# qwerty35/swarm_simulator

Hardware: AMD Instinct MI355X
Metric: agent-trajectories/sec (RBP plan: SFC+RSFC+QP) (higher is better)
Workload: dtype f64

## Files before the change

__graft_entry__.py:

```python
import os
import subprocess
import sys

ROOT = os.path.dirname(os.path.abspath(__file__))
if ROOT not in sys.path:
    sys.path.insert(0, ROOT)


def build() -> None:
    env = dict(os.environ)
    env.setdefault("PYTORCH_ROCM_ARCH", "gfx950")
    subprocess.check_call(["make", "-C", os.path.join(ROOT, "swarm_simulator_amd", "csrc"), "all", "prof", "dev", "chain"], env=env)
    subprocess.check_call(["make", "-C", os.path.join(ROOT, "oracle"), "all"], env=env)
    rocm = os.environ.get("ROCM_PATH", "/opt/rocm")
    if os.path.exists(os.path.join(rocm, "include", "rccl", "rccl.h")):
        try:
            subprocess.check_call(["make", "-C", os.path.join(ROOT, "swarm_simulator_amd", "csrc", "rccl"), "all", f"ROCM={rocm}"], env=env)
        except subprocess.CalledProcessError as e:
            print("build: WARNING: lib/librbp_rccl.so (the optional RCCL exchange hook) did not build:", e)
    else:
        print("build: no RCCL headers under", rocm, "-- lib/librbp_rccl.so (the optional RCCL exchange hook) is not built")
    import swarm_simulator_amd
    from swarm_simulator_amd import host, planner
    host.lib()
    L = planner.lib()
    for name in planner.EXPORTED_SYMBOLS:
        getattr(L, name)
    print("build ok:", L.rbp_version().decode())


def smoke() -> None:
    import numpy as np
    from swarm_simulator_amd import host, planner
    from swarm_simulator_amd.types import Param
    from tests import oracle_lib as O

    if planner.lib().rbp_device_count() < 1:
        raise RuntimeError("smoke(): no HIP device visible; the RBP path has no CPU fallback")
    p = Param.test_sweep()
    m = host.load_mission("mission_64agents_15.json").subset([0, 16, 32, 48, 8, 24, 40, 56])
    w = host.load_world("map1.bt", p)
    init = host.ecbs_plan(w, m, p)
    ref, gpu = init.clone_inputs(), init.clone_inputs()
    rc, _ = O.corridor_update(w, m, p, ref)
    assert rc == 0
    cor = planner.Corridor(w, m, p)
    assert cor.update(False, gpu), cor.last_error
    assert np.array_equal(ref.sfc_box, gpu.sfc_box) and np.array_equal(ref.sfc_count, gpu.sfc_count)
    assert np.array_equal(ref.rsfc_normal.view(np.uint32), gpu.rsfc_normal.view(np.uint32))
    rc, rep = O.planner_update(m, p, ref)
    assert rc == 0
    pl = planner.RBPPlanner(m, p)
    assert pl.update(False, gpu), pl.last_error
    err = float(np.abs(ref.ctrl - gpu.ctrl).max())
    rel = abs(ref.total_cost - gpu.total_cost) / max(1.0, abs(ref.total_cost))
    print(f"smoke: N={m.qn} M={gpu.M} cost gpu={gpu.total_cost:.9f} oracle={ref.total_cost:.9f} "
          f"ctrl sup-err={err:.2e} rel cost err={rel:.2e}")
    assert err < 1e-5 and rel < 1e-7, (err, rel)
    print("smoke ok")


if __name__ == "__main__":
    build()
    if len(sys.argv) > 1 and sys.argv[1] == "smoke":
        smoke()
```

swarm_simulator_amd/csrc/kernels/knot_lds.inc:

```
#pragma once
#include "knot_panel_layout.h"

#define KL_LD 38
#define KL_LDU 50
#define KL_I 40
#ifndef KL_XCH
#define KL_XCH 6
#endif
typedef __attribute__((address_space(3))) double kl_lds;
typedef __attribute__((address_space(3))) int kl_ldsi;
typedef double kl_d2 __attribute__((ext_vector_type(2)));
typedef __attribute__((address_space(3))) kl_d2 kl_lds2;
typedef double kl_d4 __attribute__((ext_vector_type(4)));

__host__ __device__ constexpr int kl_area_doubles(int nk) {
    return ((nk + 1) * KL_LDU + (nk + 1) * KL_LD + KL_I + 1) & ~1;
}

template <int NK>
struct KlArea {
    static constexpr int NT = (NK + 15) / 16;
    static constexpr int C = 0, CSZ = (NK + 1) * KL_LDU;
    static constexpr int MX = CSZ, MXSZ = (NK + 1) * KL_LD;
    static constexpr int I = MX + MXSZ;
// ... 459 lines not shown

template <int NK, bool WAIT>
__device__ __forceinline__ void kl_inverse_panels(kl_d4 (&n)[KlPanels<NK>::TILES], const kl_lds* C, int lane, kl_ldsi* P, int pbase) {
    constexpr int NT = KlPanels<NK>::NT, NP = KlPanels<NK>::NP;
    const int li = lane & 15, lk = lane >> 4;
#pragma unroll
    for (int ti = 0; ti < NT; ++ti)
#pragma unroll
        for (int tj = 0; tj <= ti; ++tj)
#pragma unroll
            for (int g = 0; g < 4; ++g) n[kp_lower(ti, tj)][g] = (ti == tj && lk + 4 * g == li) ? 1.0 : 0.0;
#pragma unroll
    for (int p = 0; p < NP; ++p) {
        const int tc = kp_panel_tile(p), q = kp_panel_reg(p);
        if (WAIT) kl_await_opaque(P, pbase + p + 1);
        const kl_lds* img = C + kp_img_off(NK, p);
        const kl_lds* bl = img + kp_img_entry(KP_W * p, 0);
        const double l10 = bl[4], l32 = bl[14];
        const kl_d2 r2 = *(const kl_lds2*)(bl + 8), r3 = *(const kl_lds2*)(bl + 12);
        kl_d2 raw[NT][2];
        kl_rows_load<NK>(raw, img, tc, li);
        const double l20 = r2[0], l21 = r2[1], l30 = r3[0], l31 = r3[1];
        const double k10 = -l10, k21 = -l21, k32 = -l32;
        const double k20 = __builtin_fma(-l21, k10, -l20), k31 = __builtin_fma(-l32, k21, -l31);
        const double k30 = __builtin_fma(-l32, k20, __builtin_fma(-l31, k10, -l30));
        double a[NT], b[NT];
#pragma unroll
        for (int t = 0; t < NT; ++t)
            if (t >= tc) {
                const double L[4] = {raw[t][0][0], raw[t][0][1], raw[t][1][0], raw[t][1][1]};
                double G[4];
                G[3] = -L[3];
                G[2] = -__builtin_fma(L[3], k32, L[2]);
                G[1] = -__builtin_fma(L[3], k31, __builtin_fma(L[2], k21, L[1]));
                G[0] = -__builtin_fma(L[3], k30, __builtin_fma(L[2], k20, __builtin_fma(L[1], k10, L[0])));
                if (t == tc) {
                    const int ar = KP_T * t + li - KP_W * p;
                    G[0] = kl_pick(ar >= 4, G[0], kl_pick(ar == 1, k10, kl_pick(ar == 2, k20, kl_pick(ar == 3, k30, 0.0))));
                    G[1] = kl_pick(ar >= 4, G[1], kl_pick(ar == 2, k21, kl_pick(ar == 3, k31, 0.0)));
                    G[2] = kl_pick(ar >= 4, G[2], kl_pick(ar == 3, k32, 0.0));
                    G[3] = kl_pick(ar >= 4, G[3], 0.0);
                }
                a[t] = kl_sel4(G, lk);
            }
#pragma unroll
        for (int tj = 0; tj < NT; ++tj)
            if (tj <= tc) b[tj] = n[kp_lower(tc, tj)][q];
#pragma unroll
        for (int ti = 0; ti < NT; ++ti)
#pragma unroll
            for (int tj = 0; tj <= ti; ++tj)
                if (ti >= tc && tj <= tc) n[kp_lower(ti, tj)] = __builtin_amdgcn_mfma_f64_16x16x4f64(a[ti], b[tj], n[kp_lower(ti, tj)], 0, 0, 0);
    }
}

template <int NK>
__device__ __forceinline__ void kl_tiles_scatter(const kl_d4 (&n)[KlPanels<NK>::TILES], kl_lds* MX, int lane) {
    constexpr int NT = KlPanels<NK>::NT;
    const int li = lane & 15, lk = lane >> 4;
#pragma unroll
    for (int ti = 0; ti < NT; ++ti)
#pragma unroll
        for (int tj = 0; tj < NT; ++tj)
#pragma unroll
            for (int g = 0; g < 4; ++g) {
                if (KP_T * ti + 4 * g >= NK) continue;
                const int col = KP_T * ti + lk + 4 * g, row = KP_T * tj + li;
                const bool in = (KP_T * tj + KP_T <= NK || row < NK) && (KP_T * ti + 4 * g + 4 <= NK || col < NK);
                MX[in ? row * KL_LD + col : NK * KL_LD + li] = tj <= ti ? n[kp_lower(ti, tj)][g] : 0.0;
            }
    kl_sync();
}
template <int NK>
__device__ __forceinline__ void kl_row_load(double (&m)[NK], const kl_lds* MX, int r, bool act) {
    const kl_lds* row = MX + (act ? r : NK) * KL_LD;
#pragma unroll
    for (int k = 0; k + 1 < NK; k += 2) {
        const kl_d2 t = *(const kl_lds2*)(row + k);
        m[k] = t[0], m[k + 1] = t[1];
    }
    if (NK & 1) m[NK - 1] = row[NK - 1];
}

template <int NK, bool FOLLOW>
__device__ __forceinline__ double kl_inverse_rows(double (&m)[NK], const kl_lds* C, const kl_lds* I, kl_lds* MX, int r, bool act, kl_ldsi* P, int pbase,
                                                  kl_ldsi* Mdone = nullptr, int done_value = 0) {
    if constexpr (kl_panel_path(NK)) {
        kl_d4 n[KlPanels<NK>::TILES];
        kl_inverse_panels<NK, FOLLOW>(n, C, r, P, pbase);
        kl_tiles_scatter<NK>(n, MX, r);
        if (kl_fused_path(NK)) {
            if (FOLLOW) kl_await_opaque(P, pbase + NK + 1);
            const double dinv = I[act ? r : 0];
            __builtin_amdgcn_fence(__ATOMIC_RELEASE, "wavefront");
            if (FOLLOW) kl_publish(Mdone, done_value);
            kl_row_load<NK>(m, MX, r, act);
            return dinv;
        }
        kl_row_load<NK>(m, MX, r, act);
        kl_sync();
        if (FOLLOW) kl_await_opaque(P, pbase + NK + 1);
        const double dinv = I[act ? r : 0];
        if (FOLLOW) kl_publish(Mdone, done_value);
        return dinv;
    } else {
#pragma unroll
        for (int k = 0; k < NK; ++k) m[k] = (k == r) ? 1.0 : 0.0;
        if (FOLLOW)
            kl_follow_LinvT<NK>(m, C, I, P, pbase);
        else
            kl_row_times_LinvT<NK>(m, C, I);
        if (FOLLOW) kl_await_opaque(P, pbase + NK + 1);
        const double dinv = I[act ? r : 0];
        kl_store_rows<NK>(m, MX, r, act);
        if (FOLLOW) kl_publish(Mdone, done_value);
        return dinv;
    }
}

#include "knot_subst.h"
template <int NK>
__device__ __forceinline__ void kl_forward_step(kl_lds* base, __attribute__((address_space(1))) double* z_out, double rhs_r, double e0, double e1, double e2, int r) {
    using A = KlArea<NK>;
    using F = KfSlots<NK>;
    static_assert(F::CSZ == A::CSZ, "knot_subst.h out of step with KlArea");
    kl_lds *C = base + A::C, *MX = base + A::MX, *I = base + A::I;
    const int rr = r < NK ? r : 0, g3 = 3 * (rr / 3);
    ks_step_forward<NK, true>((const kl_lds*)MX, I[rr], rhs_r, true, e0, e1, e2, C + F::A, C + F::Z, C + F::V, C + F::PS, r, g3, rr, [] { kl_sync(); },
                              [&](double z) { *z_out = z; });
}
template <int NK>
__device__ __forceinline__ double kl_middle_step(kl_lds* base, double v, int r) {
    using A = KlArea<NK>;
    using F = KfSlots<NK>;
    kl_lds* C = base + A::C;
    const int rr = r < NK ? r : 0;
    return ks_step_middle<NK, true>((const kl_lds*)(base + A::MX), (const kl_lds*)(base + A::I + rr), v, C + F::A, C + F::Z, C + F::PS, r, rr, [] { kl_sync(); });
}
```

swarm_simulator_amd/csrc/kernels/qp.hip:

```cpp
#include <algorithm>
#include <type_traits>
#include <vector>

#include "rbp_dev.h"

#pragma clang fp contract(fast)

#include "knot_lds.inc"
#include "common/ipm_rows.h"
#include "common/reduce_order.h"

#ifndef QP_THREADS
#define QP_THREADS 512
#endif
#define QP_MAX_ITERS 80
#ifndef QP_WARM_TAU
#define QP_WARM_TAU 1e-3
#endif
#ifndef QP_MU0
#define QP_MU0 3e-1
#endif
#ifndef QP_ROW_UNROLL
#define QP_ROW_UNROLL 2
#endif
#ifndef QP_ROW_PF
#define QP_ROW_PF 0
#endif
#ifndef QP_ROW_BLK
#define QP_ROW_BLK (QP_THREADS >= 512 ? 0 : 4)
#endif
#define QG(p) ((__attribute__((address_space(1))) double*)(p))
#define QGC(p) ((__attribute__((address_space(1))) const double*)(p))
#define QGF(p) ((__attribute__((address_space(1))) const float*)(p))
#ifndef QP_FAR_SLACK
#define QP_FAR_SLACK 0.7
#endif
#ifndef QP_SIGMA_POW
#define QP_SIGMA_POW 3
#endif
#ifndef QP_NBHD_GAMMA
#define QP_NBHD_GAMMA 1e-3
#endif
#ifndef QP_NBHD_BACKOFF
#define QP_NBHD_BACKOFF 0.8
#endif
#ifndef QP_STEP_FRAC
#define QP_STEP_FRAC 0.997
#endif
#ifndef QP_SFLOOR
#define QP_SFLOOR 1e-1
#endif
#ifndef QP_WAVES_PER_EU
#define QP_WAVES_PER_EU 2
#endif
#ifndef QP_CHAIN_PRIO
#define QP_CHAIN_PRIO 3
#endif
#ifndef QP_STAGE_BUFS
#define QP_STAGE_BUFS (QP_THREADS >= 512 ? 3 : 2)
#endif
#ifndef QP_STAGE_REGS
#define QP_STAGE_REGS (QP_THREADS >= 512 ? 0 : 2)
#endif
#ifndef QP_MID_FOLLOW
#define QP_MID_FOLLOW (QP_THREADS >= 512)
#endif
#ifndef QP_LF_PACKED
#define QP_LF_PACKED (QP_THREADS >= 512 ? 0 : 1)
#endif
#ifndef QP_FWD_IN_FACTOR
#ifdef QP_TRACE
#define QP_FWD_IN_FACTOR 0
#else
#define QP_FWD_IN_FACTOR 1
#endif
#endif
#if QP_FWD_IN_FACTOR && KL_FUSED_UPDATE && KL_PANEL && KL_PANEL_MIN_NK <= 36
#define QP_FWD36 1
#else
#define QP_FWD36 0
#endif
#ifndef QP_EARLY_TRIES
#define QP_EARLY_TRIES 2
#endif
#ifndef QP_EARLY_TOL
#define QP_EARLY_TOL 1e-6
#endif
#include "lh_layout.h"
#include "knot_factor_layout.h"
#define PL_NC 256
#define PL_PMAX 160
#define PL_PBIG 192
__host__ __device__ inline int polish_pmax(int nk) { return nk <= 36 ? 112 : PL_PMAX; }
__host__ __device__ inline size_t polish_s_doubles(int nj) { return std::max((size_t)PL_NC * PL_NC, ipm::k0g_doubles(nj)); }
__host__ __device__ inline size_t polish_ws_doubles(int nj, int nk) {
    return 18 * (size_t)nj + 2 + ipm::k0g_doubles(nj) + PL_NC * 14 + polish_s_doubles(nj) + 8 + lhp_size(PL_PBIG) + 4 * 6 * PL_PBIG + 3 * (size_t)nj * nk;
}
__host__ __device__ inline int polish_lds_doubles(int nk) {
    const int pm = polish_pmax(nk);
    return lhp_size(pm) + 3 * PL_NC + 3 * pm + (pm + 2 * PL_NC + 8) / 2 + 8;
}

namespace {
using namespace ipm;

#include "qp_base.inc"
#include "qp_polish_types.inc"
#include "qp_rows.inc"
#include "qp_newton.inc"
#include "qp_wave_factor.inc"
#include "qp_wave_solve.inc"
#include "qp_tiled.inc"
#include "qp_entries.inc"
#include "qp_polish.inc"
#include "qp_batch.inc"

__global__ __launch_bounds__(QP_THREADS, QP_WAVES_PER_EU) void qp_batch_kernel(DevSession S, double* ws_base, size_t ws_stride, int passes,
                                                               int biter, int nbmax, int lds_doubles) {
    const int mission = S.qp_order ? __builtin_amdgcn_readfirstlane(S.qp_order[blockIdx.x]) : (int)blockIdx.x;
    const long long t_start = wall_clock64();
    __shared__ DevSession S_lds;
    if (threadIdx.x == 0) S_lds = S;
    __syncthreads();
    mission_tables(&S_lds, ws_base, ws_stride, mission, nbmax);
    int stop_it = -1, stop_l = 0;
    for (int it = 0; it < passes && stop_it < 0; ++it)
        for (int l = 0; l < biter; ++l) {
            const double far_R = (it == 0 && S.p.polish && S.p.far_slack > 0.0) ? S.p.far_slack : 1e300;
            const int again = qp_batch_body(S, ws_base, ws_stride, mission, l, nbmax, (int)(l == 0), lds_doubles, it, far_R);
            __threadfence_block();
            __syncthreads();
            if (again) {
                stop_it = it, stop_l = l;
                break;
            }
        }
    if (stop_it >= 0) qp_finish_schedule(&S_lds, ws_base, ws_stride, mission, passes, biter, nbmax, lds_doubles, stop_it, stop_l);
    if (S.qp_cost && threadIdx.x == 0) S.qp_cost[mission] = (unsigned long long)(wall_clock64() - t_start) + 1;
}

__global__ __launch_bounds__(256) void qp_order_kernel(DevSession S) {
    const int k = blockIdx.x * blockDim.x + threadIdx.x;
    if (k >= S.K) return;
    const unsigned long long c = S.qp_cost[k];
    int rank = 0;
    bool valid = c != 0;
    for (int o = 0; o < S.K; ++o) {
        const unsigned long long co = S.qp_cost[o];
        valid = valid && co != 0;
        rank += (co > c || (co == c && o < k)) ? 1 : 0;
    }
    if (valid)
        S.qp_order[rank] = k;
    else
        S.qp_order[k] = k;
}

}

#ifndef QP_SUFFIX
#define QP_SUFFIX _w2
#endif
#define QP_CAT2(a, b) a##b
#define QP_CAT(a, b) QP_CAT2(a, b)
size_t QP_CAT(planner_workspace_bytes, QP_SUFFIX)(int N, int M, int batch_size_eff) {
    return (ws_doubles(N, M, batch_size_eff) * sizeof(double) + 255) & ~size_t(255);
}

static size_t qp_lds_bytes(int bs, int M) {
    const int nk = 9 * bs;
    const int nkw = std::min(nk, 36);
    size_t lds = sizeof(double) * (2 * (size_t)((nk + 15) & ~15) + QP_THREADS + 32) + 16;
// ... 34 lines not shown
```

swarm_simulator_amd/csrc/kernels/qp_newton.inc:

```

__device__ void apply_FT(const QpDims& d, const QpWs& w, const double* cvec, double* out, double scale) {
    const int oq = d.oq, nu = 3 * d.nb;
    for (int it = threadIdx.x; it < d.nj * nu; it += QP_THREADS) {
        const int j = it / nu + 1, u = it % nu;
        const double* xr = cvec + (size_t)u * oq + 6 * j;
        const double* xl = cvec + (size_t)u * oq + 6 * (j - 1) + 3;
        const double* L = w.Lk + 9 * j;
#pragma unroll
        for (int e = 0; e < 3; ++e)
            out[(size_t)(j - 1) * d.nk + u * 3 + e] = scale * (xr[e] + L[0 + e] * xl[0] + L[3 + e] * xl[1] + L[6 + e] * xl[2]);
    }
}
__device__ void apply_F(const QpDims& d, const QpWs& w, const double* du, double* dx) {
    const int oq = d.oq, nu = 3 * d.nb;
    for (int it = threadIdx.x; it < d.nj * nu; it += QP_THREADS) {
        const int j = it / nu + 1, u = it % nu;
        const double* uu = du + (size_t)(j - 1) * d.nk + u * 3;
        const double* L = w.Lk + 9 * j;
        const double u0 = uu[0], u1 = uu[1], u2 = uu[2];
        double* o = dx + (size_t)u * oq + 6 * (j - 1) + 3;
        o[0] = L[0] * u0 + L[1] * u1 + L[2] * u2;
        o[1] = L[3] * u0 + L[4] * u1 + L[5] * u2;
        o[2] = L[6] * u0 + L[7] * u1 + L[8] * u2;
        o[3] = u0, o[4] = u1, o[5] = u2;
// ... 62 lines not shown
    }
}
__device__ void rhs_from_acc(const RowCtx& c, bool corrector, double sigma_mu) {
    const QpDims& d = c.d;
    const QpWs& w = c.w;
    const int oq = d.oq, nu = 3 * d.nb;
    for (int it = threadIdx.x; it < d.nj * nu; it += QP_THREADS) {
        const int j = it / nu + 1, u = it % nu, a = u / 3, k = u % 3;
        double g[6];
#pragma unroll
        for (int q = 0; q < 6; ++q) {
            const int j6 = 6 * (j - 1) + 3 + q;
            const double* ac = w.cpacc + (size_t)a * oq + j6;
            const size_t ncp = (size_t)d.nb * oq;
            const double gv = corrector ? ac[k * ncp] - sigma_mu * ac[(3 + k) * ncp] : ac[(6 + k) * ncp];
            g[q] = gv;
        }
        const double* L = w.Lk + 9 * j;
        const size_t o0 = (size_t)(j - 1) * d.nk + u * 3;
#pragma unroll
        for (int e = 0; e < 3; ++e) w.rhs[o0 + e] = w.rbase[o0 + e] + g[3 + e] + L[0 + e] * g[0] + L[3 + e] * g[1] + L[6 + e] * g[2];
    }
}

__device__ inline double sym3s(const double* S, size_t stride, int k, int l) {
    const int a = k < l ? k : l, b = k < l ? l : k;
    return S[(size_t)(a == 0 ? b : (a == 1 ? 2 + b : 5)) * stride];
}
__device__ inline double sym3(const double* S, int k, int l) {
    const int a = k < l ? k : l, b = k < l ? l : k;
    return S[a == 0 ? b : (a == 1 ? 2 + b : 5)];
}

struct AsmArgs {
    const double *cpacc, *pwgt, *Lk, *Dk;
    const float* normals;
    double* Td;
    int N, M, nb, first, oq, ldb;
};
__device__ __forceinline__ AsmArgs uni(const AsmArgs& A) {
    return AsmArgs{uni(A.cpacc), uni(A.pwgt), uni(A.Lk), uni(A.Dk), uni(A.normals), uni(A.Td), uni(A.N), uni(A.M), uni(A.nb), uni(A.first), uni(A.oq), uni(A.ldb)};
}

__device__ __forceinline__ void assemble_load(const AsmArgs& A, const double* Ssum, int j, int a, int b, int k, int l, double (&Sv)[6]) {
    const int nb = A.nb, oq = A.oq;
#pragma unroll
    for (int p = 0; p < 6; ++p) {
        const int j6 = 6 * (j - 1) + 3 + p;
        double sv;
        if (a == b) {
            sv = Ssum ? sym3(Ssum + ((size_t)a * oq + j6) * 6, k, l) : sym3s(A.cpacc + (size_t)a * oq + j6, (size_t)nb * oq, k, l);
        } else {
            const int lo = a < b ? a : b, hi = a < b ? b : a, seg = j6 / 6;
            const float* nv = A.normals + (pair_index(A.N, A.first + lo, A.first + hi) * A.M + seg) * 3;
            sv = -A.pwgt[(size_t)(lo * nb - lo * (lo + 1) / 2 + (hi - lo - 1)) * oq + j6] * (double)nv[k] * (double)nv[l];
        }
        Sv[p] = sv;
    }
}
__device__ __forceinline__ void assemble_store(const AsmArgs& A, int j, int a, int b, int k, int l, const double (&Sv)[6], bool lower_only) {
    const int lb = A.ldb;
    const double* L = A.Lk + 9 * j;
    double* out = A.Td + (size_t)(j - 1) * lb * lb + (size_t)(a * 9 + k * 3) * lb + b * 9 + l * 3;
#pragma unroll
    for (int e = 0; e < 3; ++e)
#pragma unroll
        for (int f = 0; f < 3; ++f) {
            double acc = Sv[0] * L[e] * L[f] + Sv[1] * L[3 + e] * L[3 + f] + Sv[2] * L[6 + e] * L[6 + f];
            if (e == f) acc += Sv[3 + e];
            if (a == b && k == l) acc += A.Dk[9 * j + 3 * e + f];
            if (!(lower_only && a == b && k == l && e > f)) out[(size_t)e * lb + f] = acc;
        }
}
__device__ __forceinline__ void assemble_item(const AsmArgs& A, const double* Ssum, int j, int r, bool lower_only = false) {
    const int nb = A.nb;
    const int a = r / (nb * 9), b = (r / 9) % nb, k = (r / 3) % 3, l = r % 3;
    if (lower_only && (a > b || (a == b && k > l))) return;
    double Sv[6];
    assemble_load(A, Ssum, j, a, b, k, l, Sv);
    assemble_store(A, j, a, b, k, l, Sv, lower_only);
}

#define ASML_DOUBLES(nk, nb) ((nk) * KL_LD + (nb) * 36 + 3 * (nb) * ((nb) - 1) + 3 * (nb) * ((nb) - 1) + 8)
template <bool TO_GLOBAL, class NextFn, class DoneFn>
__device__ __forceinline__ void assemble_knots_lds(const AsmArgs& A, double* scratch, NextFn next, DoneFn done) {
    const int nb = A.nb, oq = A.oq, nk = 9 * nb, npb = nb * (nb - 1) / 2, n3 = 3 * nb, per = n3 * (n3 + 1) / 2;
    const int lane = threadIdx.x & 63;
    const size_t ncp = (size_t)nb * oq;
    kl_lds* Timg = (kl_lds*)scratch;
    kl_lds* Sin = Timg + nk * KL_LD;
    kl_lds* Pw = Sin + nb * 36;
    kl_lds* Nr = Pw + 6 * npb;
    int tA[2], tB[2], ntile = 0;
#pragma unroll
    for (int u = 0; u < 2; ++u) {
        const int t = lane + 64 * u, tc = t < per ? t : 0;
        int ai = (int)(((2 * n3 + 1) - sqrtf((float)((2 * n3 + 1) * (2 * n3 + 1) - 8 * tc))) * 0.5f);
        if (ai * n3 - ai * (ai - 1) / 2 > tc) ai--;
        if ((ai + 1) * n3 - (ai + 1) * ai / 2 <= tc) ai++;
        tA[u] = ai, tB[u] = ai + tc - (ai * n3 - ai * (ai - 1) / 2);
        if (t < per) ntile = u + 1;
    }
    const int row0 = (2 * lane) / nk, col0 = (2 * lane) % nk, drow = 128 / nk, dcol = 128 % nk;
    size_t nr_off = 0;
    if (lane < 6 * npb) {
        const int pw = lane / 6, sg = (lane / 3) % 2, c3 = lane % 3;
        int lo = 0, rest = pw;
        while (rest >= nb - 1 - lo) rest -= nb - 1 - lo, lo++;
        const int hi = lo + 1 + rest;
        nr_off = (pair_index(A.N, A.first + lo, A.first + hi) * A.M + sg) * 3 + c3;
    }
    for (int j = next(); j >= 0; j = next()) {
        const int jn = j + 1, j60 = 6 * j + 3;
        for (int idx = lane; idx < nb * 36; idx += 64) {
            const int a = idx / 36, e = (idx / 6) % 6, pp = idx % 6;
            Sin[idx] = A.cpacc[(size_t)e * ncp + (size_t)a * oq + j60 + pp];
        }
        for (int idx = lane; idx < 6 * npb; idx += 64) Pw[idx] = A.pwgt[(size_t)(idx / 6) * oq + j60 + idx % 6];
        if (lane < 6 * npb) Nr[lane] = (double)A.normals[nr_off + (size_t)j * 3];
        double L[9], Dk[9];
#pragma unroll
        for (int e = 0; e < 9; ++e) L[e] = A.Lk[9 * jn + e], Dk[e] = A.Dk[9 * jn + e];
        kl_sync();
#pragma unroll
        for (int u = 0; u < 2; ++u) {
            if (u < ntile) {
                const int Ai = tA[u], Bi = tB[u], a = Ai / 3, k = Ai % 3, b = Bi / 3, l = Bi % 3;
                double Sv[6];
                if (a == b) {
                    const int kk = k < l ? k : l, ll = k < l ? l : k, sym = kk == 0 ? ll : (kk == 1 ? 2 + ll : 5);
#pragma unroll
                    for (int pp = 0; pp < 6; ++pp) Sv[pp] = Sin[(a * 6 + sym) * 6 + pp];
                } else {
                    const int pw = a * nb - a * (a + 1) / 2 + (b - a - 1);
#pragma unroll
                    for (int pp = 0; pp < 6; ++pp) Sv[pp] = -Pw[pw * 6 + pp] * Nr[(pw * 2 + (pp >= 3)) * 3 + k] * Nr[(pw * 2 + (pp >= 3)) * 3 + l];
                }
#pragma unroll
                for (int e = 0; e < 3; ++e)
#pragma unroll
                    for (int f = 0; f < 3; ++f) {
                        double acc = Sv[0] * L[e] * L[f] + Sv[1] * L[3 + e] * L[3 + f] + Sv[2] * L[6 + e] * L[6 + f];
                        if (e == f) acc += Sv[3 + e];
                        if (Ai == Bi) acc += Dk[3 * e + f];
                        Timg[(3 * Ai + e) * KL_LD + 3 * Bi + f] = acc;
                        Timg[(3 * Bi + f) * KL_LD + 3 * Ai + e] = acc;
                    }
            }
        }
        kl_sync();
        if (TO_GLOBAL) {
            double* Tg = A.Td + (size_t)j * nk * nk;
            if ((nk & 1) == 0) {
                int r = row0, k2 = col0;
                for (int idx = lane; idx < nk * nk / 2; idx += 64) {
                    if (k2 + 1 >= r) *(kl_d2*)(Tg + 2 * idx) = *(const kl_lds2*)(Timg + r * KL_LD + k2);
                    r += drow, k2 += dcol;
                    if (k2 >= nk) k2 -= nk, r++;
                }
            } else {
                for (int idx = lane; idx < nk * nk; idx += 64) Tg[idx] = Timg[(idx / nk) * KL_LD + idx % nk];
            }
        }
        done(j);
        kl_sync();
    }
}
__device__ __noinline__ void fasm_fetch(AsmArgs Av, double* scratch_v, int jv) {
    typedef __attribute__((address_space(1))) const void gvoid;
    typedef __attribute__((address_space(3))) void lvoid;
    typedef __attribute__((address_space(3))) char lchar;
    const AsmArgs A = uni(Av);
    double* scratch = uni(scratch_v);
    const int j = __builtin_amdgcn_readfirstlane(jv);
    const int nb = A.nb, oq = A.oq, nk = 9 * nb, npb = nb * (nb - 1) / 2, lane = threadIdx.x & 63, j60 = 6 * j + 3;
    const size_t ncp = (size_t)nb * oq;
    lchar* Sin = (lchar*)((kl_lds*)scratch + nk * KL_LD);
    lchar* Pw = Sin + (size_t)nb * 36 * 8;
    lchar* Nr = Pw + (size_t)6 * npb * 8;
    asm volatile("s_waitcnt lgkmcnt(0)" ::: "memory");
    for (int c = 0; c * 64 < nb * 72; ++c) {
        const int dw = c * 64 + lane, idx = dw >> 1, a = idx / 36, e = (idx / 6) % 6, pp = idx % 6;
        if (dw < nb * 72)
            __builtin_amdgcn_global_load_lds((gvoid*)((const unsigned*)(A.cpacc + (size_t)e * ncp + (size_t)a * oq + j60 + pp) + (dw & 1)), (lvoid*)(Sin + c * 256), 4, 0, 0);
    }
    for (int c = 0; c * 64 < npb * 12; ++c) {
        const int dw = c * 64 + lane, idx = dw >> 1;
        if (dw < npb * 12)
            __builtin_amdgcn_global_load_lds((gvoid*)((const unsigned*)(A.pwgt + (size_t)(idx / 6) * oq + j60 + idx % 6) + (dw & 1)), (lvoid*)(Pw + c * 256), 4, 0, 0);
    }
    if (lane < 6 * npb) {
        const int pw = lane / 6, sg = (lane / 3) % 2, c3 = lane % 3;
        int lo = 0, rest = pw;
        while (rest >= nb - 1 - lo) rest -= nb - 1 - lo, lo++;
        const int hi = lo + 1 + rest;
        const size_t off = (pair_index(A.N, A.first + lo, A.first + hi) * A.M + sg + j) * 3 + c3;
        __builtin_amdgcn_global_load_lds((gvoid*)(A.normals + off), (lvoid*)Nr, 4, 0, 0);
    }
}
__device__ __noinline__ void fasm_tiles(AsmArgs Av, double* scratch_v, int jv) {
    const AsmArgs A = uni(Av);
    double* scratch = uni(scratch_v);
    const int j = __builtin_amdgcn_readfirstlane(jv);
    const int nb = A.nb, nk = 9 * nb, npb = nb * (nb - 1) / 2, n3 = 3 * nb, per = n3 * (n3 + 1) / 2, lane = threadIdx.x & 63, jn = j + 1;
    kl_lds* Timg = (kl_lds*)scratch;
    const kl_lds* Sin = Timg + nk * KL_LD;
    const kl_lds* Pw = Sin + nb * 36;
    const __attribute__((address_space(3))) float* Nr = (const __attribute__((address_space(3))) float*)(Pw + 6 * npb);
    double L[9], Dk[9];
#pragma unroll
    for (int e = 0; e < 9; ++e) L[e] = A.Lk[9 * jn + e], Dk[e] = A.Dk[9 * jn + e];
    asm volatile("s_waitcnt vmcnt(0)" ::: "memory");
    kl_sync();
    for (int u = 0; u * 64 < per; ++u) {
        const int t = lane + 64 * u;
        if (t < per) {
            int Ai = (int)(((2 * n3 + 1) - sqrtf((float)((2 * n3 + 1) * (2 * n3 + 1) - 8 * t))) * 0.5f);
            if (Ai * n3 - Ai * (Ai - 1) / 2 > t) Ai--;
            if ((Ai + 1) * n3 - (Ai + 1) * Ai / 2 <= t) Ai++;
            const int Bi = Ai + t - (Ai * n3 - Ai * (Ai - 1) / 2);
            const int a = Ai / 3, k = Ai % 3, b = Bi / 3, l = Bi % 3;
            double Sv[6];
            if (a == b) {
                const int kk = k < l ? k : l, ll = k < l ? l : k, sym = kk == 0 ? ll : (kk == 1 ? 2 + ll : 5);
#pragma unroll
                for (int pp = 0; pp < 6; ++pp) Sv[pp] = Sin[(a * 6 + sym) * 6 + pp];
            } else {
                const int pw = a * nb - a * (a + 1) / 2 + (b - a - 1);
#pragma unroll
                for (int pp = 0; pp < 6; ++pp)
                    Sv[pp] = -Pw[pw * 6 + pp] * (double)Nr[(pw * 2 + (pp >= 3)) * 3 + k] * (double)Nr[(pw * 2 + (pp >= 3)) * 3 + l];
            }
#pragma unroll
            for (int e = 0; e < 3; ++e)
#pragma unroll
                for (int f = 0; f < 3; ++f) {
                    double acc = Sv[0] * L[e] * L[f] + Sv[1] * L[3 + e] * L[3 + f] + Sv[2] * L[6 + e] * L[6 + f];
                    if (e == f) acc += Sv[3 + e];
                    if (Ai == Bi) acc += Dk[3 * e + f];
                    Timg[(3 * Ai + e) * KL_LD + 3 * Bi + f] = acc;
                    Timg[(3 * Bi + f) * KL_LD + 3 * Ai + e] = acc;
                }
        }
    }
    kl_sync();
}
__device__ void assemble_blocks_lds(const AsmArgs& A, int nj, double* lds) {
    const int wave = threadIdx.x >> 6, NW = QP_THREADS / 64;
    int j = wave - NW;
    assemble_knots_lds<true>(A, lds + (size_t)wave * ASML_DOUBLES(9 * A.nb, A.nb), [&] { j += NW; return j < nj ? j : -1; }, [](int) {});
}

__device__ inline AsmArgs asm_args(const RowCtx& c) {
    return AsmArgs{c.w.cpacc, c.w.pwgt, c.w.Lk, c.w.Dk, c.normals, c.w.Td, c.d.N, c.d.M, c.d.nb, c.d.first, c.d.oq, c.d.ldb};
}

__device__ void assemble_blocks(const RowCtx& c, double* lds) {
    const QpDims& d = c.d;
    const QpWs& w = c.w;
    const int nk = d.nk, oq = d.oq, nb = d.nb, lb = d.ldb;
    const AsmArgs A = asm_args(c);
    const bool in_lds = nb * oq * 6 <= c.lds_avail;
    if (in_lds) {
        for (int it = threadIdx.x; it < nb * oq * 6; it += QP_THREADS) lds[it] = w.cpacc[(size_t)(it % 6) * (nb * oq) + it / 6];
        __syncthreads();
    }
    const int per_knot = nb * nb * 9;
    for (int it = threadIdx.x; it < d.nj * per_knot; it += QP_THREADS) assemble_item(A, in_lds ? lds : nullptr, it / per_knot + 1, it % per_knot);
    if (d.nj > 1 && nk > 36 && 3 * lb * (lb + 2) > c.lds_avail) {
        const size_t noff = (size_t)(d.nj - 1) * lb * lb;
        for (size_t it = threadIdx.x; it < noff; it += QP_THREADS) {
            const int j = (int)(it / ((size_t)lb * lb)) + 1;
            const int rr = (int)(it % ((size_t)lb * lb)) / lb, cc = (int)(it % ((size_t)lb * lb)) % lb;
            double v = 0;
            if (rr / 3 == cc / 3 && rr < nk && cc < nk) v = w.Ek[9 * j + 3 * (cc % 3) + (rr % 3)];
            w.To[it] = v;
        }
    }
}
```

swarm_simulator_amd/csrc/kernels/qp_wave_factor.inc:

```

__device__ __forceinline__ int twist_mid(int nj) { return nj / 2; }

#define ASM_WAVE0 4
#define ASM_HELPERS (QP_THREADS / 64 > ASM_WAVE0 ? QP_THREADS / 64 - ASM_WAVE0 : 0)
#ifndef QP_FOLLOW_ASM
#define QP_FOLLOW_ASM (ASM_HELPERS == 0)
#endif
#define ASMF_READY(cnt, h) ((kl_ldsi*)((cnt) + 76 + (h)))
__device__ __forceinline__ void wait_blocks(int* cnt, int i) {
    while (__hip_atomic_load(cnt + i, __ATOMIC_RELAXED, __HIP_MEMORY_SCOPE_WORKGROUP) < ASM_HELPERS) __builtin_amdgcn_s_sleep(2);
    __builtin_amdgcn_fence(__ATOMIC_ACQUIRE, "workgroup");
}

typedef double d4 __attribute__((ext_vector_type(4)));

template <int NK>
__device__ __forceinline__ bool chol_rows(double (&a)[NK], double& dinv) {
    bool ok = true;
    const int r = threadIdx.x & 63;
    dinv = 1.0;
#pragma unroll
    for (int c = 0; c < NK; ++c) {
        const double dcc = rl(a[c], c);
        if (!(dcc > 0)) ok = false;
        const double inv = fast_rsqrt(dcc);
        dinv = (r == c) ? inv : dinv;
        a[c] *= inv;
#pragma unroll
        for (int k = c + 1; k < NK; ++k) a[k] -= a[c] * rl(a[c], k);
    }
    return ok;
}

#if QP_LF_PACKED
#define KF_SLOT(NK) kf_stride(NK)
#define KF_ELEM(NK, r, k) kf_elem(NK, r, k)
#define KF_DINV(NK) kf_dinv(NK)
#else
static_assert(KL_I == 40, "kf_sq_stride (knot_factor_layout.h) restates KL_I");
#define KF_SLOT(NK) kf_sq_stride(NK)
#define KF_ELEM(NK, r, k) kf_sq_elem(NK, r, k)
#define KF_DINV(NK) kf_sq_dinv(NK)
#endif
static_assert(KF_SLOT(9) + 15 <= 2 * 81 && KF_SLOT(18) + 15 <= 2 * 324 && KF_SLOT(27) + 15 <= 2 * 729 && KF_SLOT(36) + 15 <= 2 * 1296,
              "a knot's slot and the doubles in front of the first one fit the region carve() gives QpWs::Lf");

__device__ __forceinline__ void coupling_coef(const QpWs& w, int j, int dir, int rr, double& e0, double& e1, double& e2) {
    const __attribute__((address_space(1))) double* E = QGC(w.Ek) + 9 * (dir > 0 ? j + 1 : j);
    e0 = dir > 0 ? E[rr % 3] : E[3 * (rr % 3)], e1 = dir > 0 ? E[3 + rr % 3] : E[3 * (rr % 3) + 1],
    e2 = dir > 0 ? E[6 + rr % 3] : E[3 * (rr % 3) + 2];
}

template <int NK>
__device__ __forceinline__ bool knot_ldl(const QpWs& w, int j, bool minus_u, kl_lds* base, int r, bool act, int rr, kl_ldsi* P, int pbase,
                                         const kl_lds* Timg = nullptr, kl_ldsi* consumed = nullptr, int consumed_value = 0) {
    using A = KlArea<NK>;
    kl_lds *C = base + A::C, *I = base + A::I, *U = base + A::C;
    if constexpr (kl_panel_path(NK)) {
        if (Timg)
            return kl_knot_panels<NK, true>([&](int mx, int mn) { return (double)Timg[mn * KL_LD + mx]; },
                                      [&] {
                                          kl_sync();
                                          if (consumed) kl_publish(consumed, consumed_value);
                                      },
                                      minus_u, C, I, r, P, pbase);
        const double* Tg = w.Td + (size_t)j * NK * NK;
        return kl_knot_panels<NK, false>([&](int mx, int mn) { return Tg[mn * NK + mx]; }, [] {}, minus_u, C, I, r, P, pbase);
    }
    double a[NK];
    if (Timg) {
#pragma unroll
        for (int k = 0; k < NK; ++k) a[k] = Timg[k * KL_LD + rr];
        kl_sync();
        if (consumed) kl_publish(consumed, consumed_value);
    } else {
        const double* Tg = w.Td + (size_t)j * NK * NK;
#pragma unroll
        for (int k = 0; k < NK; ++k) a[k] = Tg[k * NK + rr];
    }
    if (minus_u) {
#pragma unroll
        for (int k = 0; k < NK; ++k) a[k] -= U[rr * KL_LDU + k];
        kl_sync();
    }
    return kl_ldl<NK>(a, C, I, r, act, P, pbase);
}

template <int NK>
__device__ __forceinline__ bool knot_ldl_add(const QpWs& w, int j, kl_d4 (&s)[KlPanels<NK>::TILES], kl_lds* base, int r, kl_ldsi* P, int pbase,
                                             const kl_lds* Timg = nullptr, kl_ldsi* consumed = nullptr, int consumed_value = 0) {
    using A = KlArea<NK>;
    kl_lds *C = base + A::C, *I = base + A::I;
    if (Timg)
        return kl_knot_panels_add<NK, true>(s, [&](int mx, int mn) { return (double)Timg[mn * KL_LD + mx]; },
                                            [&] {
                                                kl_sync();
                                                if (consumed) kl_publish(consumed, consumed_value);
                                            },
                                            C, I, r, P, pbase);
    const double* Tg = w.Td + (size_t)j * NK * NK;
    return kl_knot_panels_add<NK, false>(s, [&](int mx, int mn) { return Tg[mn * NK + mx]; }, [] {}, C, I, r, P, pbase);
}
template <int NK>
__device__ __forceinline__ void fused_coupling_coef(const QpWs& w, int j, int dir, int lane, double (&cf)[KlPanels<NK>::NT][3]) {
    const __attribute__((address_space(1))) double* E = QGC(w.Ek) + 9 * (dir > 0 ? j + 1 : j);
    kl_fused_coef<NK>(cf, lane, [&](int row, int q) { return dir > 0 ? E[3 * q + row % 3] : E[3 * (row % 3) + q]; });
}

template <int NK, bool FOLLOW>
__device__ __forceinline__ void knot_inverse(const QpWs& w, int j, kl_lds* base, int r, bool act, kl_ldsi* P, int pbase, int& seen, kl_ldsi* Mdone,
                                             int done_value) {
    using A = KlArea<NK>;
    kl_lds *C = base + A::C, *MX = base + A::MX, *I = base + A::I;
    double m[NK];
    const double dinv = kl_inverse_rows<NK, FOLLOW>(m, C, I, MX, r, act, P, pbase, Mdone, done_value);
    __attribute__((address_space(1))) double* Mg = QG(w.Lf + (size_t)j * KF_SLOT(NK));
    if (FOLLOW && QP_FOLLOW_ASM) asm volatile("s_waitcnt vmcnt(0)" ::: "memory");
    if (act) {
        __attribute__((address_space(1))) double* row = Mg + KF_ELEM(NK, r, 0);
        if ((NK & 1) == 0) {
#pragma unroll
            for (int k = 0; k < NK; k += 2)
                if (k + 1 >= r) *(__attribute__((address_space(1))) kl_d2*)(row + k) = kl_d2{m[k], m[k + 1]};
        } else {
#pragma unroll
            for (int k = 0; k < NK; ++k)
                if (k >= r) row[k] = m[k];
        }
        Mg[KF_DINV(NK) + r] = dinv;
    }
}

#if defined(QP_PROFILE) && !defined(QP_LHSTATS) && !defined(QP_SOLVE_TIMERS)
#define CHAIN_TW(cnt, slot) ((__attribute__((address_space(3))) unsigned long long*)((cnt) + 96) + ((slot) - 25))
#define CHAIN_T0 long long ct_ = wall_clock64()
#define CHAIN_T(slot)                                                                                                                              \
    do {                                                                                                                                           \
        const long long t_ = wall_clock64();                                                                                                       \
        __hip_atomic_fetch_add(CHAIN_TW(cnt, slot), (dir > 0 && r == 0) ? (unsigned long long)(t_ - ct_) : 0ull, __ATOMIC_RELAXED, __HIP_MEMORY_SCOPE_WORKGROUP); \
        ct_ = t_;                                                                                                                                  \
    } while (0)
#define CHAIN_FLUSH()                                                                                   \
    do {                                                                                                \
        kl_sync();                                                                                      \
        if (w.prof && dir > 0 && r == 0)                                                                \
            for (int k_ = 25; k_ < 28; ++k_) w.prof[k_] += (double)(long long)*CHAIN_TW(cnt, k_);       \
        if (QP_FWD_IN_FACTOR && w.prof && dir > 0 && r == 0) w.prof[29] += (double)(long long)*CHAIN_TW(cnt, 29); \
    } while (0)
#else
#define CHAIN_T0
#define CHAIN_T(slot)
#define CHAIN_FLUSH()
#endif
#define CHAIN_SYNC(cnt, h) ((kl_ldsi*)((cnt) + 64 + 2 * (h)))
#define ASM_CONSUMED(cnt, h) ((kl_ldsi*)((cnt) + 72 + (h)))

static_assert((QP_FWD36 != 0) == (QP_FWD_IN_FACTOR && kl_fused_path(36)), "QP_FWD36 (qp.hip) out of step with kl_fused_path");
template <int NK>
__device__ __forceinline__ void wave_forward_step(const QpWs& w, kl_lds* base, int jp, double rhs_r, double e0, double e1, double e2, int r) {
    kl_forward_step<NK>(base, QG(w.rhs) + (size_t)jp * NK + (r < NK ? r : 0), rhs_r, e0, e1, e2, r);
}
template <int NK>
__device__ __forceinline__ void wave_forward_fetch(const QpWs& w, int j, int dir, bool first, int r, double& rhs_r, double& e0, double& e1, double& e2) {
    const int rr = r < NK ? r : 0;
    rhs_r = QGC(w.rhs)[(size_t)j * NK + rr];
    coupling_coef(w, first ? j : j - dir, dir, rr, e0, e1, e2);
    e0 = first ? 0.0 : e0, e1 = first ? 0.0 : e1, e2 = first ? 0.0 : e2;
}

template <int NK>
__device__ __forceinline__ bool wave_factor_chain(const QpDims& d, const QpWs& w, int j0, int count, int dir, double* ldsW, int* cnt, int h) {
    using A = KlArea<NK>;
    kl_lds* base = (kl_lds*)ldsW;
    kl_lds *MX = base + A::MX, *I = base + A::I, *U = base + A::C;
    kl_ldsi *P = CHAIN_SYNC(cnt, h), *Mdone = P + 1;
    const int r = threadIdx.x & 63;
    const bool act = r < NK;
    const int rr = act ? r : 0;
    bool ok = true;
    int seen = 0, seen_img = 0;
    if constexpr (kl_fused_path(NK)) {
        double cf[KlPanels<NK>::NT][3];
        [[maybe_unused]] double f_rhs = 0, f_e0 = 0, f_e1 = 0, f_e2 = 0;
        for (int i = 0, j = j0; i < count; ++i, j += dir) {
            CHAIN_T0;
            kl_d4 s[KlPanels<NK>::TILES];
            kl_tiles_zero<NK>(s);
            if (i > 0) {
                kl_await(Mdone, i, seen);
                CHAIN_T(27);
                kl_fused_update<NK>(s, MX, I, r, cf);
            }
            CHAIN_T(25);
            if (QP_FWD_IN_FACTOR) {
                if (i > 0) wave_forward_step<NK>(w, base, j - dir, f_rhs, f_e0, f_e1, f_e2, r);
                CHAIN_T(29);
            }
            if (QP_FOLLOW_ASM)
                kl_await(ASMF_READY(cnt, h), i + 1, seen_img);
            else
// ... 103 lines not shown
            v -= e0 * V0[g3] + e1 * V0[g3 + 1] + e2 * V0[g3 + 2];
        }
        if (mid + 1 < d.nj) {
            double e0, e1, e2;
            coupling_coef(w, mid + 1, -1, rr, e0, e1, e2);
            v -= e0 * V1[g3] + e1 * V1[g3 + 1] + e2 * V1[g3 + 2];
        }
        const double x = kl_middle_step<NK>(bl, v, r);
        QG(w.rhs)[(size_t)mid * NK + rr] = x;
    }
    return ok;
}

template <int NK, int ROLE>
__device__ __forceinline__ bool twisted_factor(const QpDims& d, const QpWs& w, int* flag, double* lds, const AsmArgs* asmb) {
    const int wave = (ROLE == 0 || ROLE == 2) ? (threadIdx.x >> 6) & 1 : 4, mid = twist_mid(d.nj);
    const int nl = mid, nr = d.nj - 1 - mid, SF = nl > nr ? nl : nr;
    constexpr int AREA = KlArea<NK>::SIZE;
    int* cnt = (int*)(lds + 2 * AREA);
    static_assert((QP_MAX_M - 1) / 2 + 1 <= 64, "cnt[0..SF] must end below CHAIN_SYNC (cnt + 64): sessions with M > QP_MAX_M are refused");
    if (threadIdx.x == 0) *flag = 0;
    __syncthreads();
    bool ok = true;
    for (int i = threadIdx.x; i < 2 * AREA + 64; i += QP_THREADS) lds[i] = 0.0;
    __syncthreads();
    if (ROLE == 0) {
        __builtin_amdgcn_s_setprio(QP_CHAIN_PRIO);
        if (wave == 0 && mid > 0) ok = wave_factor_chain<NK>(d, w, 0, mid, +1, lds, cnt, 0);
        if (wave == 1 && nr > 0) ok = wave_factor_chain<NK>(d, w, d.nj - 1, nr, -1, lds + AREA, cnt, 1);
        if (wave == 1) __builtin_amdgcn_s_setprio(0);
    }
    if (ROLE == 1) {
        const AsmArgs A = *asmb;
        const int hw = (threadIdx.x >> 6) - ASM_WAVE0, side = hw & 1, par = hw >> 1;
        double* scratch = lds + 2 * AREA + 128 + (size_t)hw * ASML_DOUBLES(NK, (NK / 9));
        int i = par - 2;
        kl_ldsi* consumed = ASM_CONSUMED(cnt, side);
        int seen_c = 0;
        assemble_knots_lds<false>(
            A, scratch,
            [&] {
                for (i += 2; i <= SF; i += 2) {
                    const bool work = i < SF ? (side ? i < nr : i < nl) : side == 0;
                    if (work) {
                        if (i >= 2) kl_await(consumed, i - 1, seen_c);
                        return i < SF ? (side ? d.nj - 1 - i : i) : mid;
                    }
                    if ((threadIdx.x & 63) == 0)
                        __hip_atomic_fetch_add(cnt + i, i < SF ? ASM_HELPERS / 2 : 0, __ATOMIC_RELAXED, __HIP_MEMORY_SCOPE_WORKGROUP);
                }
                return -1;
            },
            [&](int) {
                __builtin_amdgcn_fence(__ATOMIC_RELEASE, "workgroup");
                if ((threadIdx.x & 63) == 0)
                    __hip_atomic_fetch_add(cnt + i, i < SF ? ASM_HELPERS / 2 : ASM_HELPERS, __ATOMIC_RELAXED, __HIP_MEMORY_SCOPE_WORKGROUP);
            });
    }
    if (ROLE == 2) {
        const int count = wave == 0 ? nl : nr, j0 = wave == 0 ? 0 : d.nj - 1, dir = wave == 0 ? +1 : -1;
        kl_lds* base = (kl_lds*)(lds + wave * AREA);
        kl_ldsi *P = CHAIN_SYNC(cnt, wave), *Mdone = P + 1;
        const int r = threadIdx.x & 63;
        int seen = 0;
        if (QP_FOLLOW_ASM) {
            const AsmArgs A = *asmb;
            double* scratch = lds + 2 * AREA + 128 + (size_t)wave * ASML_DOUBLES(NK, (NK / 9));
            kl_ldsi *ready = ASMF_READY(cnt, wave), *consumed = ASM_CONSUMED(cnt, wave);
            const int total = count + (wave == 0 ? 1 : 0);
            int seen_c = 0;
            auto blk = [&](int n) { return n < count ? j0 + n * dir : mid; };
            auto make = [&](int n) {
                if (n > 0) kl_await(consumed, n, seen_c);
                fasm_tiles(A, scratch, blk(n));
                __builtin_amdgcn_fence(__ATOMIC_RELEASE, "workgroup");
                kl_publish(ready, n + 1);
                if (n + 1 < total) fasm_fetch(A, scratch, blk(n + 1));
            };
            if (total > 0) {
                fasm_fetch(A, scratch, blk(0));
                make(0);
            }
            for (int i = 0; i < count; ++i) {
                knot_inverse<NK, true>(w, j0 + i * dir, base, r, r < NK, P, i * (NK + 1), seen, Mdone, i + 1);
                if (i + 1 < total) make(i + 1);
            }
        } else {
            for (int i = 0; i < count; ++i) knot_inverse<NK, true>(w, j0 + i * dir, base, r, r < NK, P, i * (NK + 1), seen, Mdone, i + 1);
        }
    }
    if (!ok && (threadIdx.x & 63) == 0) atomicExch(flag, 1);
    __threadfence_block();
    __syncthreads();
    if (*flag) return false;
    if (ROLE == 0 && wave == 0) {
        if (!wave_factor_mid<NK>(d, w, lds, lds + AREA, cnt, SF) && threadIdx.x == 0) *flag = 1;
        __builtin_amdgcn_s_setprio(0);
    }
    if (QP_MID_FOLLOW && ROLE == 2 && wave == 0) {
        const int r = threadIdx.x & 63;
        int seen = 0;
        kl_ldsi* P = CHAIN_SYNC(cnt, 2);
        knot_inverse<NK, true>(w, mid, (kl_lds*)lds, r, r < NK, P, 0, seen, P + 1, 1);
    }
    __threadfence_block();
    __syncthreads();
    return *flag == 0;
}
```

Measured before the change: 199,700.

## Assemble next knot image before storing inverse rows; stage L/Dk via LDS

In the follower-wave chain, the next knot's assembly (make) now runs inside knot_inverse right after the done flag is published, before the inverse rows are stored to global memory. This lets the next image be built while the global stores drain, and the vmcnt(0) wait before the stores is dropped when this path is active. For batches of 4, the Lk/Dk coefficients are also fetched straight into LDS with global_load_lds alongside the other scratch loads instead of as per-lane scalar global loads. The change adds a callback template parameter and layout static_asserts, and it risks reordering hazards between the outstanding stores and the scratch reuse.

After: 201,300, median of 6. Within noise of the previous version (+0.8%).

```diff
diff --git a/__graft_entry__.py b/__graft_entry__.py
--- a/__graft_entry__.py
+++ b/__graft_entry__.py
@@ -10,7 +10,7 @@
 def build() -> None:
     env = dict(os.environ)
     env.setdefault("PYTORCH_ROCM_ARCH", "gfx950")
-    subprocess.check_call(["make", "-C", os.path.join(ROOT, "swarm_simulator_amd", "csrc"), "all", "prof", "dev", "chain"], env=env)
+    subprocess.check_call(["make", "-C", os.path.join(ROOT, "swarm_simulator_amd", "csrc"), "all", "prof", "dev", "chain", "imagelate"], env=env)
     subprocess.check_call(["make", "-C", os.path.join(ROOT, "oracle"), "all"], env=env)
     rocm = os.environ.get("ROCM_PATH", "/opt/rocm")
     if os.path.exists(os.path.join(rocm, "include", "rccl", "rccl.h")):
diff --git a/swarm_simulator_amd/csrc/kernels/asm_scratch_layout.h b/swarm_simulator_amd/csrc/kernels/asm_scratch_layout.h
--- /dev/null
+++ b/swarm_simulator_amd/csrc/kernels/asm_scratch_layout.h
@@ -0,0 +1,16 @@
+#pragma once
+#ifndef ASL_FN
+#define ASL_FN __host__ __device__ inline
+#endif
+
+ASL_FN constexpr int asl_pairs(int nb) { return nb * (nb - 1) / 2; }
+ASL_FN constexpr int asl_sin(int nk, int ld) { return nk * ld; }
+ASL_FN constexpr int asl_pw(int nk, int nb, int ld) { return asl_sin(nk, ld) + nb * 36; }
+ASL_FN constexpr int asl_nr(int nk, int nb, int ld) { return asl_pw(nk, nb, ld) + 6 * asl_pairs(nb); }
+ASL_FN constexpr int asl_nr_doubles(int nb) { return 3 * nb * (nb - 1); }
+ASL_FN constexpr int asl_nr_floats(int nb) { return 6 * asl_pairs(nb); }
+ASL_FN constexpr int asl_total(int nk, int nb, int ld) { return asl_nr(nk, nb, ld) + asl_nr_doubles(nb) + 8; }
+#define ASL_LD_DOUBLES 18
+ASL_FN constexpr int asl_ld(int nk, int nb, int ld) { return asl_nr(nk, nb, ld) + (asl_nr_floats(nb) + 1) / 2; }
+ASL_FN constexpr int asl_dk(int nk, int nb, int ld) { return asl_ld(nk, nb, ld) + 9; }
+ASL_FN constexpr bool asl_ld_fits(int nb) { return (asl_nr_floats(nb) + 1) / 2 + ASL_LD_DOUBLES <= asl_nr_doubles(nb); }
diff --git a/swarm_simulator_amd/csrc/kernels/knot_lds.inc b/swarm_simulator_amd/csrc/kernels/knot_lds.inc
--- a/swarm_simulator_amd/csrc/kernels/knot_lds.inc
+++ b/swarm_simulator_amd/csrc/kernels/knot_lds.inc
@@ -565,9 +565,12 @@
     if (NK & 1) m[NK - 1] = row[NK - 1];
 }
 
-template <int NK, bool FOLLOW>
+struct KlNoop {
+    __device__ void operator()() const {}
+};
+template <int NK, bool FOLLOW, class AnnouncedFn = KlNoop>
 __device__ __forceinline__ double kl_inverse_rows(double (&m)[NK], const kl_lds* C, const kl_lds* I, kl_lds* MX, int r, bool act, kl_ldsi* P, int pbase,
-                                                  kl_ldsi* Mdone = nullptr, int done_value = 0) {
+                                                  kl_ldsi* Mdone = nullptr, int done_value = 0, AnnouncedFn&& announced = AnnouncedFn{}) {
     if constexpr (kl_panel_path(NK)) {
         kl_d4 n[KlPanels<NK>::TILES];
         kl_inverse_panels<NK, FOLLOW>(n, C, r, P, pbase);
@@ -577,6 +580,7 @@
             const double dinv = I[act ? r : 0];
             __builtin_amdgcn_fence(__ATOMIC_RELEASE, "wavefront");
             if (FOLLOW) kl_publish(Mdone, done_value);
+            announced();
             kl_row_load<NK>(m, MX, r, act);
             return dinv;
         }
diff --git a/swarm_simulator_amd/csrc/kernels/qp.hip b/swarm_simulator_amd/csrc/kernels/qp.hip
--- a/swarm_simulator_amd/csrc/kernels/qp.hip
+++ b/swarm_simulator_amd/csrc/kernels/qp.hip
@@ -80,6 +80,9 @@
 #else
 #define QP_FWD36 0
 #endif
+#ifndef QP_IMAGE_FIRST
+#define QP_IMAGE_FIRST 1
+#endif
 #ifndef QP_EARLY_TRIES
 #define QP_EARLY_TRIES 2
 #endif
@@ -88,6 +91,7 @@
 #endif
 #include "lh_layout.h"
 #include "knot_factor_layout.h"
+#include "asm_scratch_layout.h"
 #define PL_NC 256
 #define PL_PMAX 160
 #define PL_PBIG 192
diff --git a/swarm_simulator_amd/csrc/kernels/qp_newton.inc b/swarm_simulator_amd/csrc/kernels/qp_newton.inc
--- a/swarm_simulator_amd/csrc/kernels/qp_newton.inc
+++ b/swarm_simulator_amd/csrc/kernels/qp_newton.inc
@@ -168,6 +168,9 @@
 }
 
 #define ASML_DOUBLES(nk, nb) ((nk) * KL_LD + (nb) * 36 + 3 * (nb) * ((nb) - 1) + 3 * (nb) * ((nb) - 1) + 8)
+static_assert(ASML_DOUBLES(36, 4) == asl_total(36, 4, KL_LD) && ASML_DOUBLES(27, 3) == asl_total(27, 3, KL_LD) && ASML_DOUBLES(18, 2) == asl_total(18, 2, KL_LD) &&
+                  ASML_DOUBLES(9, 1) == asl_total(9, 1, KL_LD),
+              "image | Sin | Pw | Nr | 8: asm_scratch_layout.h states the offsets");
 template <bool TO_GLOBAL, class NextFn, class DoneFn>
 __device__ __forceinline__ void assemble_knots_lds(const AsmArgs& A, double* scratch, NextFn next, DoneFn done) {
     const int nb = A.nb, oq = A.oq, nk = 9 * nb, npb = nb * (nb - 1) / 2, n3 = 3 * nb, per = n3 * (n3 + 1) / 2;
@@ -252,6 +255,9 @@
         kl_sync();
     }
 }
+__host__ __device__ constexpr bool fasm_ld_in_lds(int nb) { return QP_IMAGE_FIRST && kl_fused_path(9 * nb) && asl_ld_fits(nb); }
+static_assert(asl_ld_fits(4) && !asl_ld_fits(3) && asl_dk(36, 4, KL_LD) + 9 == asl_nr(36, 4, KL_LD) + asl_nr_doubles(4) && 2 * ASL_LD_DOUBLES <= 64,
+              "L and Dk of a batch of 4 fill the Nr region behind the normals' floats exactly; one dword per lane fetches them");
 __device__ __noinline__ void fasm_fetch(AsmArgs Av, double* scratch_v, int jv) {
     typedef __attribute__((address_space(1))) const void gvoid;
     typedef __attribute__((address_space(3))) void lvoid;
@@ -283,6 +289,11 @@
         const size_t off = (pair_index(A.N, A.first + lo, A.first + hi) * A.M + sg + j) * 3 + c3;
         __builtin_amdgcn_global_load_lds((gvoid*)(A.normals + off), (lvoid*)Nr, 4, 0, 0);
     }
+    if (fasm_ld_in_lds(nb) && lane < 2 * ASL_LD_DOUBLES) {
+        const bool isL = lane < ASL_LD_DOUBLES;
+        const unsigned* src = (const unsigned*)((isL ? A.Lk : A.Dk) + 9 * (j + 1)) + (isL ? lane : lane - ASL_LD_DOUBLES);
+        __builtin_amdgcn_global_load_lds((gvoid*)src, (lvoid*)((lchar*)((kl_lds*)scratch + asl_ld(nk, nb, KL_LD))), 4, 0, 0);
+    }
 }
 __device__ __noinline__ void fasm_tiles(AsmArgs Av, double* scratch_v, int jv) {
     const AsmArgs A = uni(Av);
@@ -293,11 +304,19 @@
     const kl_lds* Sin = Timg + nk * KL_LD;
     const kl_lds* Pw = Sin + nb * 36;
     const __attribute__((address_space(3))) float* Nr = (const __attribute__((address_space(3))) float*)(Pw + 6 * npb);
+    const bool ld_lds = fasm_ld_in_lds(nb);
     double L[9], Dk[9];
-#pragma unroll
-    for (int e = 0; e < 9; ++e) L[e] = A.Lk[9 * jn + e], Dk[e] = A.Dk[9 * jn + e];
+    if (!ld_lds) {
+#pragma unroll
+        for (int e = 0; e < 9; ++e) L[e] = A.Lk[9 * jn + e], Dk[e] = A.Dk[9 * jn + e];
+    }
     asm volatile("s_waitcnt vmcnt(0)" ::: "memory");
     kl_sync();
+    if (ld_lds) {
+        const kl_lds* LD = Timg + asl_ld(nk, nb, KL_LD);
+#pragma unroll
+        for (int e = 0; e < 9; ++e) L[e] = LD[e], Dk[e] = LD[9 + e];
+    }
     for (int u = 0; u * 64 < per; ++u) {
         const int t = lane + 64 * u;
         if (t < per) {
diff --git a/swarm_simulator_amd/csrc/kernels/qp_wave_factor.inc b/swarm_simulator_amd/csrc/kernels/qp_wave_factor.inc
--- a/swarm_simulator_amd/csrc/kernels/qp_wave_factor.inc
+++ b/swarm_simulator_amd/csrc/kernels/qp_wave_factor.inc
@@ -7,6 +7,7 @@
 #define QP_FOLLOW_ASM (ASM_HELPERS == 0)
 #endif
 #define ASMF_READY(cnt, h) ((kl_ldsi*)((cnt) + 76 + (h)))
+__host__ __device__ constexpr bool qp_image_first(int nk) { return QP_IMAGE_FIRST && QP_FOLLOW_ASM && kl_fused_path(nk); }
 __device__ __forceinline__ void wait_blocks(int* cnt, int i) {
     while (__hip_atomic_load(cnt + i, __ATOMIC_RELAXED, __HIP_MEMORY_SCOPE_WORKGROUP) < ASM_HELPERS) __builtin_amdgcn_s_sleep(2);
     __builtin_amdgcn_fence(__ATOMIC_ACQUIRE, "workgroup");
@@ -107,15 +108,15 @@
     kl_fused_coef<NK>(cf, lane, [&](int row, int q) { return dir > 0 ? E[3 * q + row % 3] : E[3 * (row % 3) + q]; });
 }
 
-template <int NK, bool FOLLOW>
+template <int NK, bool FOLLOW, class AnnouncedFn = KlNoop>
 __device__ __forceinline__ void knot_inverse(const QpWs& w, int j, kl_lds* base, int r, bool act, kl_ldsi* P, int pbase, int& seen, kl_ldsi* Mdone,
-                                             int done_value) {
+                                             int done_value, AnnouncedFn&& announced = AnnouncedFn{}) {
     using A = KlArea<NK>;
     kl_lds *C = base + A::C, *MX = base + A::MX, *I = base + A::I;
     double m[NK];
-    const double dinv = kl_inverse_rows<NK, FOLLOW>(m, C, I, MX, r, act, P, pbase, Mdone, done_value);
+    const double dinv = kl_inverse_rows<NK, FOLLOW>(m, C, I, MX, r, act, P, pbase, Mdone, done_value, announced);
     __attribute__((address_space(1))) double* Mg = QG(w.Lf + (size_t)j * KF_SLOT(NK));
-    if (FOLLOW && QP_FOLLOW_ASM) asm volatile("s_waitcnt vmcnt(0)" ::: "memory");
+    if (FOLLOW && QP_FOLLOW_ASM && !qp_image_first(NK)) asm volatile("s_waitcnt vmcnt(0)" ::: "memory");
     if (act) {
         __attribute__((address_space(1))) double* row = Mg + KF_ELEM(NK, r, 0);
         if ((NK & 1) == 0) {
@@ -385,8 +386,14 @@
                 make(0);
             }
             for (int i = 0; i < count; ++i) {
-                knot_inverse<NK, true>(w, j0 + i * dir, base, r, r < NK, P, i * (NK + 1), seen, Mdone, i + 1);
-                if (i + 1 < total) make(i + 1);
+                if constexpr (qp_image_first(NK)) {
+                    knot_inverse<NK, true>(w, j0 + i * dir, base, r, r < NK, P, i * (NK + 1), seen, Mdone, i + 1, [&] {
+                        if (i + 1 < total) make(i + 1);
+                    });
+                } else {
+                    knot_inverse<NK, true>(w, j0 + i * dir, base, r, r < NK, P, i * (NK + 1), seen, Mdone, i + 1);
+                    if (i + 1 < total) make(i + 1);
+                }
             }
         } else {
             for (int i = 0; i < count; ++i) knot_inverse<NK, true>(w, j0 + i * dir, base, r, r < NK, P, i * (NK + 1), seen, Mdone, i + 1);
```
